# sshaoshuai/PointRCNN

Measured on NVIDIA B200. Metric: scenes/sec RPN backbone fwd (16384 pts), higher is better.
Workload: dtype f32 (tf32 tensor-core MLP, fp32 accumulate)

## Files before the change

include/pointrcnn_b200.h:

```cpp
#ifndef POINTRCNN_B200_H_
#define POINTRCNN_B200_H_

#include <stddef.h>
#include <stdint.h>

#ifdef __cplusplus
extern "C" {
#endif

#define PRB_ABI_VERSION 5
#if defined(__GNUC__)
#define PRB_API __attribute__((visibility("default")))
#else
#define PRB_API
#endif

PRB_API int prb_abi_version(void);
PRB_API const char *prb_last_error(void);
PRB_API unsigned long long prb_launch_count(void);

typedef struct prb_options {
    int fps_cluster;
    int fps_prune;
    int fps_threads;
// ... 78 lines not shown

PRB_API size_t prb_mlp_packed_bytes(int num_layers, int c_in, const int *c_out);
PRB_API int prb_mlp_pack_weights(int num_layers, int c_in, const int *c_out, const float *const *w, void *dst);

PRB_API int prb_sa_group_mlp_max(int b, int n, int npoint, int nsample, int c_feat, const float *xyz,
                         const float *new_xyz, const float *feats_pm, const int *idx,
                         const prb_mlp_desc *mlp, float *out, int out_stride_c, int out_c_off,
                         void *stream);

PRB_API int prb_fp_interp_mlp(int b, int n, int m, int c_known, int c_skip, const float *known_pm,
                      const int *idx, const float *weight, const float *skip,
                      const prb_mlp_desc *mlp, float *out, void *stream);

PRB_API size_t prb_mlp_packed_bytes_ex(int kind, int split, int num_layers, int c_in, const int *c_out);
PRB_API int prb_mlp_pack_weights_ex(int kind, int split, int num_layers, int c_in, const int *c_out,
                                    const float *const *w, void *dst);
PRB_API size_t prb_sa_workspace_bytes(int b, int npoint, int nsample, int c_feat, int num_layers, const int *c_out);
PRB_API size_t prb_fp_workspace_bytes(int b, int n, int c_known, int c_skip, int num_layers, const int *c_out);
PRB_API size_t prb_rows_workspace_bytes(long rows, int c_in, int num_layers, const int *c_out);
PRB_API int prb_sa_group_mlp_max_ws(int b, int n, int npoint, int nsample, int c_feat, const float *xyz,
                                    const float *new_xyz, const float *feats_pm, const int *idx,
                                    const prb_mlp_desc *mlp, float *out, float *out_pm, int out_stride_c,
                                    int out_c_off, void *workspace, size_t workspace_bytes, void *stream);
PRB_API int prb_fp_interp_mlp_ws(int b, int n, int m, int c_known, int c_skip, const float *known_pm,
                                 const int *idx, const float *weight, const float *skip,
                                 const prb_mlp_desc *mlp, float *out, float *out_pm, void *workspace,
                                 size_t workspace_bytes, void *stream);
PRB_API int prb_mlp_rows(long rows, int c_in, const float *x_rows, const prb_mlp_desc *mlp, float *out_rows,
                         int out_pitch, void *workspace, size_t workspace_bytes, void *stream);
PRB_API size_t prb_rows2_workspace_bytes(long rows, int c_a, int c_b, int num_layers, const int *c_out);
PRB_API int prb_mlp_rows2(long rows, int c_a, const float *a_rows, int a_pitch, int c_b, const float *b_rows, int b_pitch,
                          const prb_mlp_desc *mlp, float *out_rows, int out_pitch, void *workspace, size_t workspace_bytes,
                          void *stream);

PRB_API int prb_decode_rpn_proposals(long n, int c, const float *xyz, const float *reg, const float *anchor_hwl,
                                     float loc_scope, float loc_bin_size, int num_head_bin, int get_xz_fine, float *out,
                                     void *stream);
PRB_API size_t prb_rpn_proposals_workspace_bytes(int b, int post_nms_top_n);
PRB_API int prb_rpn_proposals(int b, int n, const float *boxes, const float *scores, const long long *order,
                              int distance_based, int pre_nms_top_n, int post_nms_top_n, float nms_thresh, int normal_nms,
                              float *out_boxes, float *out_scores, void *workspace, size_t workspace_bytes, void *stream);

PRB_API int prb_debug_mlp_trace(long long *dst);
PRB_API int prb_debug_pipe_trace(long long *dst);
PRB_API int prb_debug_tuned_plans(int *dst, int max_entries);

// ... 53 lines not shown
```

pointrcnn_b200/csrc/mlp_dev.cuh:

```cuda
#pragma once
#include <math_constants.h>

#include "common.cuh"

namespace prb {

constexpr int TM = 128;
constexpr int KC = 32;
constexpr int A_STAGE_BYTES = TM * KC * 4;
constexpr int B_TILE_ROWS = 256;
constexpr int MAX_STAGES = 4;
constexpr int MAX_LAYERS = 3;
constexpr int MAX_NP = 512;

enum { IN_SA = 0, IN_FP = 1, IN_DIRECT = 2 };
enum { OUT_ROWS = 0, OUT_SA_MAX = 1, OUT_FP = 2 };

struct ChainParams {
    int mode_in, mode_out, num_layers;
    int nchunks[MAX_LAYERS];
    int np[MAX_LAYERS];
    int dcol[MAX_LAYERS];
    const float *w[MAX_LAYERS];
    const float *scale[MAX_LAYERS];
    int w_resident;
    int sleepy_ns;
    int sleepy;
    int a_tmem;
    int trace;
    int unit_scale;
    const float *shift[MAX_LAYERS];
    int na, nb;
    int b_stage_bytes;
    int tmem_cols;
    int gather_mode;
    int linear_last;
    int round_out;
    int nseg, seg_chunks[2], seg_width[2];
    long total_rows;
    int num_tiles;
    int n, npoint, ns, log_ns, c_feat;
    const float *xyz, *new_xyz, *feats_pm;
    const int *idx;
    int m, c_known, c_skip;
    const float *known_pm, *weight, *skip;
    const float *x_rows;
    int x_pitch;
    const float *x2_rows;
    int x2_pitch;
    float *out;
    float *out_pm;
    int c_last;
    int out_stride_c, out_c_off, out_pitch;
    int rcol[MAX_LAYERS];
    int zcol[2], zs, nslice, nbuf;
    int nb0, nb1;
    int b0_stage_bytes, b1_stage_bytes;
    int b_rows;
    int nsplit, split_w;
    int num_items;
    int rows32;
    int pool_mode;
};

__device__ __forceinline__ uint32_t s2u(const void *p) { return (uint32_t)__cvta_generic_to_shared(p); }

// ... 191 lines not shown
```

pointrcnn_b200/csrc/mlp_pipe.cu:

```cuda
#include <type_traits>

#include <map>
#include <mutex>

#include "mlp_dev.cuh"

namespace prb {

constexpr int PIPE_MAX_A = 8;
constexpr int PIPE_MAX_B = 12;

struct PipeSmem {
    uint64_t a_full[PIPE_MAX_A], a_empty[PIPE_MAX_A];
    uint64_t b0_full[PIPE_MAX_B], b0_empty[PIPE_MAX_B], b1_full[PIPE_MAX_B], b1_empty[PIPE_MAX_B];
    uint64_t r_full[2];
    uint64_t x_free;
    uint64_t ready[2][16];
    uint64_t z_full[2], z_free[2];
    uint32_t tmem_base;
    int row_src[2][TM][3];
    float row_aux[2][TM][3];
    int row_valid[2][TM];
};

__host__ __device__ inline size_t pipe_smem_bytes(int ne, int na, int nb0, int b0_bytes, int nb1, int b1_bytes, int np_total, bool pool) {
    return 1024  + (size_t)na * A_STAGE_BYTES + (size_t)nb0 * b0_bytes + (size_t)nb1 * b1_bytes +
           (size_t)2 * np_total * sizeof(float) + (pool ? (size_t)ne * (TM * POOL_STRIDE + 8 * 16) * sizeof(float) : 0) + 64;
}

__device__ __forceinline__ void bar_named(int id, int nthreads) {
    asm volatile("bar.sync %0, %1;" ::"r"(id), "r"(nthreads) : "memory");
}

struct Cursor {
    int scene, pos, adv_scene, adv_pos, period;
    __device__ __forceinline__ void init(int start, int step, int per) {
        period = per;
        scene = start / per; pos = start - scene * per;
        adv_scene = step / per; adv_pos = step - adv_scene * per;
    }
    __device__ __forceinline__ void advance() {
        scene += adv_scene; pos += adv_pos;
        if (pos >= period) { pos -= period; ++scene; }
    }
    __device__ __forceinline__ void at(int off, int &sc, int &ps) const {
        sc = scene; ps = pos + off;
        while (ps >= period) { ps -= period; ++sc; }
    }
};

// ... 149 lines not shown
template <int BASE, int N>
__device__ __forceinline__ void reg_set() {
    if (N > BASE) asm volatile("setmaxnreg.inc.sync.aligned.u32 %0;" ::"n"(N));
    else if (N < BASE) asm volatile("setmaxnreg.dec.sync.aligned.u32 %0;" ::"n"(N));
}

template <int NE, int NGW, int MINB, int MIN, int MOUT>
__global__ void __launch_bounds__((NE + NGW + 1) * 128, MINB) mlp_pipe_kernel(const __grid_constant__ ChainParams p) {
    constexpr int NTHREADS = (NE + NGW + 1) * 128;
    constexpr int REG_BASE = (65536 / (NTHREADS * MINB)) / 8 * 8 > 255 ? 255 : (65536 / (NTHREADS * MINB)) / 8 * 8;
    static_assert(128 * (RegPlan<NE, NGW, MINB>::MISC + NE * RegPlan<NE, NGW, MINB>::EPI + NGW * RegPlan<NE, NGW, MINB>::GATHER) <= NTHREADS * REG_BASE,
                  "register plan exceeds the CTA's launch allocation");
    constexpr int W_GATHER = 4 * NE, W_MISC = 4 * (NE + NGW);
    extern __shared__ uint8_t smem_raw[];
    __shared__ PipeSmem S;
    uint8_t *base = smem_raw + ((1024u - (s2u(smem_raw) & 1023u)) & 1023u);
    const int L = p.num_layers;
    auto sc_off = [&](int l) { return l == 0 ? 0 : (l == 1 ? p.np[0] : p.np[0] + p.np[1]); };
    static_assert(MAX_LAYERS == 3, "sc_off assumes at most three layers");
    const int np_total = sc_off(L - 1) + p.np[L - 1];
    uint8_t *sA = base;
    uint8_t *sB0 = sA + (size_t)p.na * A_STAGE_BYTES;
    uint8_t *sB1 = sB0 + (size_t)p.nb0 * p.b0_stage_bytes;
    float *s_scale = reinterpret_cast<float *>(sB1 + (size_t)p.nb1 * p.b1_stage_bytes);
    float *s_shift = s_scale + np_total;
    float *s_pool = s_shift + np_total;
    const int tid = threadIdx.x, warp = tid >> 5, lane = tid & 31;

    if (tid == 0) {
        for (int i = 0; i < PIPE_MAX_A; ++i) { mbar_init(s2u(&S.a_full[i]), 128); mbar_init(s2u(&S.a_empty[i]), 1); }
        for (int i = 0; i < PIPE_MAX_B; ++i) {
            mbar_init(s2u(&S.b0_full[i]), 1); mbar_init(s2u(&S.b0_empty[i]), 1);
            mbar_init(s2u(&S.b1_full[i]), 1); mbar_init(s2u(&S.b1_empty[i]), 1);
        }
        for (int i = 0; i < 2; ++i) {
            mbar_init(s2u(&S.r_full[i]), 1);
            mbar_init(s2u(&S.z_full[i]), 1); mbar_init(s2u(&S.z_free[i]), 128 * NE);
            for (int k = 0; k < 16; ++k) mbar_init(s2u(&S.ready[i][k]), 128);
        }
        mbar_init(s2u(&S.x_free), 1);
        asm volatile("fence.mbarrier_init.release.cluster;" ::: "memory");
    }
    if (warp == W_MISC + 2) tmem_alloc(s2u(&S.tmem_base), (uint32_t)p.tmem_cols);
    for (int l = 0; l < L; ++l)
        for (int i = tid; i < p.np[l]; i += NTHREADS) { s_scale[sc_off(l) + i] = p.unit_scale ? 1.f : p.scale[l][i]; s_shift[sc_off(l) + i] = p.shift[l][i]; }
    tc_fence_before();
    __syncthreads();
    tc_fence_after();
    const uint32_t tmem = S.tmem_base;
    const int brows = p.b_rows;
    const int nsplit = p.nsplit;
    const int sj = (int)blockIdx.x % nsplit;
    const int tile0 = (int)blockIdx.x / nsplit, tstep = (int)gridDim.x / nsplit;
    const int ntiles = p.num_tiles;
    const bool resident = p.w_resident != 0;
    const int lazy = NE == 1 ? p.sleepy_ns : 0;
    TraceTimer tt;
    tt.start(p.trace != 0 && blockIdx.x == 0 && (warp >= W_MISC || warp == W_GATHER || warp == 0),
             warp == W_MISC + 2 ? 0 : warp == W_MISC + 3 ? 1 : warp == W_MISC ? 2 : warp == W_MISC + 1 ? 3 : warp == W_GATHER ? 4 : 5);

    if (warp >= W_MISC) {
    reg_set<REG_BASE, RegPlan<NE, NGW, MINB>::MISC>();
    if (warp == W_MISC) {
        {
            RingPos rb = {0, 0};
            const int col0 = sj * p.split_w;
            const int width = L == 1 ? min(p.split_w, p.np[0] - col0) : p.np[0];
            const int halves = (width + brows - 1) / brows;
// ... 144 lines not shown
                                        }
                                    }
                                });
                                rb.advance(nb);
                            }
                        }
                    }
                }
            }
        }
    }
    } else if (warp >= W_GATHER) {
        reg_set<REG_BASE, RegPlan<NE, NGW, MINB>::GATHER>();
        const int gw = warp - W_GATHER;
        const int wq = gw & 3, grp = gw >> 2;
        const int r = wq * 32 + lane;
        const int j8 = lane & 7;
        const int rsub = lane >> 3;
        const int na = p.na, nch0 = p.nchunks[0];
        const int rows = p.rows32;
        RingPos ra = {0, 0};
        uint32_t cc = 0, it = 0;
        Cursor cur;
        if (MIN == IN_SA) cur.init(tile0 * (TM >> p.log_ns), tstep * (TM >> p.log_ns), p.npoint);
        else if (MIN == IN_FP) cur.init(tile0 * TM, tstep * TM, p.n);
        else cur.init(0, 0, 1);
        for (int tile = tile0; tile < ntiles; tile += tstep, ++it, cur.advance()) {
            const int R = tile * TM + r;
            const bool valid = R < rows;
            int src = -1;
            float cx = 0.f, cy = 0.f, cz = 0.f;
            int my_scene = 0, my_u = 0;
            const int par = it & 1;
            if (MIN == IN_SA) {
                int sc, pp;
                cur.at(r >> p.log_ns, sc, pp);
                if (valid) {
                    src = sc * p.n + __ldg(p.idx + R);
                    const float *ctr = p.new_xyz + ((size_t)sc * p.npoint + pp) * 3;
                    cx = __ldg(ctr); cy = __ldg(ctr + 1); cz = __ldg(ctr + 2);
                }
            } else if (MIN == IN_FP) {
                cur.at(r, my_scene, my_u);
                int m_src[3] = {0, 0, 0};
                float m_w[3] = {0.f, 0.f, 0.f};
                if (valid) {
#pragma unroll
                    for (int q = 0; q < 3; ++q) {
                        m_src[q] = my_scene * p.m + __ldg(p.idx + (size_t)R * 3 + q);
                        m_w[q] = __ldg(p.weight + (size_t)R * 3 + q);
                    }
                }
                if (grp == 0) {
                    S.row_valid[par][r] = valid;
#pragma unroll
                    for (int q = 0; q < 3; ++q) { S.row_src[par][r][q] = m_src[q]; S.row_aux[par][r][q] = m_w[q]; }
                }
                bar_named(5, 128 * NGW);
            }
            int s8[8];
            if (MIN == IN_SA) {
#pragma unroll
                for (int i = 0; i < 8; ++i) s8[i] = __shfl_sync(0xffffffffu, src, rsub + 4 * i);
            } else if (MIN == IN_DIRECT) {
#pragma unroll
                for (int i = 0; i < 8; ++i) { const int rr = tile * TM + wq * 32 + rsub + 4 * i; s8[i] = rr < rows ? rr : -1; }
            }

            for (int kc = 0; kc < nch0; ++kc, ++cc, ra.advance(na)) {
                if (NGW > 1 && (int)(cc % NGW) != grp) continue;
                int c = kc, seg = 0;
                if (p.nseg > 1 && c >= p.seg_chunks[0]) { c -= p.seg_chunks[0]; seg = 1; }
                const int k0 = c * KC;
                const int width = p.seg_width[seg];
                uint8_t *A = sA + (size_t)ra.stage * A_STAGE_BYTES;
                uint64_t *empty_bar = &S.a_empty[ra.stage];
                const uint32_t empty_par = ra.phase ^ 1;
                const bool rows_seg = (MIN == IN_DIRECT) || (MIN == IN_SA && seg == 0 && p.c_feat > 5) || (MIN == IN_FP && seg == 0);
                if (rows_seg) {
                    const int kk = k0 + 4 * j8;
                    if (MIN == IN_FP) {
// ... 48 lines not shown
                        for (int i = 0; i < 8; ++i) {
                            t[i] = make_float4(0.f, 0.f, 0.f, 0.f);
                            if (s8[i] >= 0 && kk < width) {
                                const float *sp = srcbase + (size_t)s8[i] * pitch + kk;
                                if (vec) {
                                    t[i] = __ldg((const float4 *)sp);
                                } else {
                                    float o[4];
#pragma unroll
                                    for (int q = 0; q < 4; ++q) o[q] = (kk + q < width) ? __ldg(sp + q) : 0.f;
                                    t[i] = make_float4(o[0], o[1], o[2], o[3]);
                                }
                            }
                        }
                        tt.timed(0, [&] { bwait_lazy(empty_bar, empty_par, lazy); });
#pragma unroll
                        for (int i = 0; i < 8; ++i) {
                            const int rr = wq * 32 + rsub + 4 * i;
                            float4 v = t[i];
                            v.x = to_tf32(v.x); v.y = to_tf32(v.y); v.z = to_tf32(v.z); v.w = to_tf32(v.w);
                            *reinterpret_cast<float4 *>(A + swz(rr, j8)) = v;
                        }
                    }
                } else if (MIN == IN_SA) {
                    float4 v = make_float4(0.f, 0.f, 0.f, 0.f), v2 = make_float4(0.f, 0.f, 0.f, 0.f);
                    if (valid) {
                        const float *q = p.xyz + (size_t)src * 3;
                        v.x = to_tf32(__ldg(q + 0) - cx);
                        v.y = to_tf32(__ldg(q + 1) - cy);
                        v.z = to_tf32(__ldg(q + 2) - cz);
                        const int cf = p.c_feat;
                        if (cf > 0 && cf <= 5) {
                            const float *f = p.feats_pm + (size_t)src * cf;
                            v.w = to_tf32(__ldg(f));
                            if (cf > 1) v2.x = to_tf32(__ldg(f + 1));
                            if (cf > 2) v2.y = to_tf32(__ldg(f + 2));
                            if (cf > 3) v2.z = to_tf32(__ldg(f + 3));
                            if (cf > 4) v2.w = to_tf32(__ldg(f + 4));
                        }
                    }
                    tt.timed(0, [&] { bwait_lazy(empty_bar, empty_par, lazy); });
                    *reinterpret_cast<float4 *>(A + swz(r, 0)) = v;
                    *reinterpret_cast<float4 *>(A + swz(r, 1)) = v2;
                } else if (MIN == IN_FP) {
                    const float *bsrc = p.skip + (size_t)my_scene * p.c_skip * p.n + my_u;
                    float o[32];
// ... 397 lines not shown
            if (o.mlp_ne == 2) { pl.ne = pl.ngw = 2; pl.occ = 1; }
            if (pl.ne == 2 && (o.mlp_ngw == 3 || force_ngw == 3)) pl.ngw = 3;
            const int brows = o.mlp_brows >= 32 ? o.mlp_brows : 256;
            pl.brows = brows;
            int b0_rows = L == 1 ? z : p.np[0], b1_rows = 32;
            for (int l = 1; l < L; ++l) { const int w = (l == L - 1) ? z : p.np[l]; if (w > b1_rows) b1_rows = w; }
            if (b0_rows > brows) b0_rows = brows;
            if (b1_rows > brows) b1_rows = brows;
            pl.b0_bytes = b0_rows * KC * 4; pl.b1_bytes = L > 1 ? b1_rows * KC * 4 : 0;
            const size_t budget = (size_t)(227 * 1024) / pl.occ - 1024 - sizeof(PipeSmem) - 512;
            bool ok = false;
            pl.resident = 0;
            if (o.mlp_resident) {
                const int halves0 = ((L == 1 ? z : p.np[0]) + brows - 1) / brows;
                int st0 = p.nchunks[0] * halves0, st1 = 0;
                for (int l = 1; l < L; ++l) {
                    const int w = (l == L - 1) ? z : p.np[l];
                    st1 += (l == L - 1 ? nslice : 1) * p.nchunks[l] * ((w + brows - 1) / brows);
                }
                if (st0 <= PIPE_MAX_B && st1 <= PIPE_MAX_B) {
                    const int na_min = k0 + 1 < PIPE_MAX_A ? (k0 + 1 > 3 ? k0 + 1 : 3) : PIPE_MAX_A;
                    for (int na = (k0 + 2 < PIPE_MAX_A ? (k0 + 2 > 3 ? k0 + 2 : 3) : PIPE_MAX_A); na >= na_min && !ok; --na) {
                        const size_t smem = pipe_smem_bytes(pl.ne, na, st0, pl.b0_bytes, st1, pl.b1_bytes, np_total,
                                                            p.mode_out == OUT_SA_MAX && !(p.ns == 16 || p.ns == 32));
                        if (smem <= budget && smem <= (size_t)max_optin) {
                            pl.na = na; pl.nb0 = st0; pl.nb1 = st1; pl.smem = smem; pl.resident = 1; ok = true;
                        }
                    }
                }
            }
            for (int nb = 3; nb >= 2 && !ok; --nb)
                for (int na = (k0 + 2 < PIPE_MAX_A ? (k0 + 2 > 3 ? k0 + 2 : 3) : PIPE_MAX_A); na >= 2 && !ok; --na) {
                    const size_t smem = pipe_smem_bytes(pl.ne, na, nb, pl.b0_bytes, L > 1 ? nb : 0, pl.b1_bytes, np_total,
                                                        p.mode_out == OUT_SA_MAX && !(p.ns == 16 || p.ns == 32));
                    if (smem <= budget && smem <= (size_t)max_optin && (nb == 2 || na >= (k0 < 4 ? k0 : 4))) {
                        pl.na = na; pl.nb0 = nb; pl.nb1 = L > 1 ? nb : 0; pl.smem = smem; ok = true;
                    }
                }
            if (!ok) continue;
            const long score = (long)pl.occ * 1000000L + nbuf * 1000L + z;
            if (score > best_score) { best_score = score; best = pl; }
        }
    }
    if (best_score < 0) return false;
    *out = best;
    return true;
}

static int launch_with_plan(ChainParams &p, const PipePlan &pl, cudaStream_t st) {
    const int L = p.num_layers;
    int col = 0;
    for (int l = 0; l + 1 < L; ++l) { p.rcol[l] = col; col += p.np[l]; }
    p.zcol[0] = col; p.zcol[1] = col + pl.zs;
    p.zs = pl.zs; p.nslice = pl.nslice; p.nbuf = pl.nbuf;
    p.tmem_cols = pl.cols;
    p.na = pl.na; p.nb0 = pl.nb0; p.nb1 = pl.nb1 > 0 ? pl.nb1 : 1;
    p.b0_stage_bytes = pl.b0_bytes; p.b1_stage_bytes = pl.b1_bytes;
    p.nsplit = pl.nsplit; p.split_w = pl.split_w;
    p.b_rows = pl.brows;
    p.w_resident = pl.resident;
    p.num_items = p.num_tiles * pl.nsplit;
    int sms = num_sms();
    if (const int v = opts().mlp_sms; v >= 1 && v < sms) sms = v;
    int grid = sms * pl.occ;
    if (grid > p.num_items) grid = p.num_items;
    grid = grid / pl.nsplit * pl.nsplit;
    if (grid < pl.nsplit) grid = pl.nsplit;
    p.trace = opts().mlp_trace ? 1 : 0;
    p.rows32 = (int)p.total_rows;
    p.pool_mode = opts().mlp_pool;
    p.sleepy_ns = opts().mlp_lazy_ns > 0 ? opts().mlp_lazy_ns : 400;
    const size_t smem = pl.smem;
#define PRB_LAUNCH_PIPE(NE, NGW, MB, MI, MO)                                                                                   \
    do {                                                                                                                       \
        PRB_CUDA(cudaFuncSetAttribute(mlp_pipe_kernel<NE, NGW, MB, MI, MO>, cudaFuncAttributeMaxDynamicSharedMemorySize, (int)smem)); \
        mlp_pipe_kernel<NE, NGW, MB, MI, MO><<<grid, (NE + NGW + 1) * 128, smem, st>>>(p);                                      \
    } while (0)
#define PRB_LAUNCH_PIPE_IO(NE, NGW, MB)                                                                    \
    do {                                                                                                   \
        const int key = p.mode_in * 3 + p.mode_out;                                                        \
        switch (key) {                                                                                     \
            case IN_SA * 3 + OUT_ROWS: PRB_LAUNCH_PIPE(NE, NGW, MB, IN_SA, OUT_ROWS); break;              \
            case IN_SA * 3 + OUT_SA_MAX: PRB_LAUNCH_PIPE(NE, NGW, MB, IN_SA, OUT_SA_MAX); break;          \
            case IN_FP * 3 + OUT_ROWS: PRB_LAUNCH_PIPE(NE, NGW, MB, IN_FP, OUT_ROWS); break;              \
            case IN_FP * 3 + OUT_FP: PRB_LAUNCH_PIPE(NE, NGW, MB, IN_FP, OUT_FP); break;                  \
            case IN_DIRECT * 3 + OUT_ROWS: PRB_LAUNCH_PIPE(NE, NGW, MB, IN_DIRECT, OUT_ROWS); break;      \
            case IN_DIRECT * 3 + OUT_SA_MAX: PRB_LAUNCH_PIPE(NE, NGW, MB, IN_DIRECT, OUT_SA_MAX); break;  \
            case IN_DIRECT * 3 + OUT_FP: PRB_LAUNCH_PIPE(NE, NGW, MB, IN_DIRECT, OUT_FP); break;          \
            default: set_error("mlp: unsupported input / output mode pair %d / %d", p.mode_in, p.mode_out); return -1; \
        }                                                                                                  \
    } while (0)
    if (pl.occ == 3) PRB_LAUNCH_PIPE(1, 1, 3, IN_SA, OUT_SA_MAX);
    else if (pl.ne == 1 && pl.ngw == 1) PRB_LAUNCH_PIPE_IO(1, 1, 2);
    else if (pl.ngw == 3) PRB_LAUNCH_PIPE_IO(2, 3, 1);
    else PRB_LAUNCH_PIPE_IO(2, 2, 1);
#undef PRB_LAUNCH_PIPE_IO
#undef PRB_LAUNCH_PIPE
    return check_launch("mlp_pipe_kernel");
}

struct TuneKey {
    int dev, mode_in, mode_out, L, ns, k0, tiles, np[3];
    bool operator<(const TuneKey &o) const { return memcmp(this, &o, sizeof(TuneKey)) < 0; }
};
static std::mutex g_tune_mu;
struct TuneVal { int choice; int nc; int code[4]; float ms[4]; };
static std::map<TuneKey, TuneVal> g_tune;

static bool tuning_allowed(cudaStream_t st) {
    const prb_options &o = opts();
    if (!o.mlp_tune || o.mlp_trace || o.mlp_occ || o.mlp_ne || o.mlp_ngw || o.mlp_zs || o.mlp_nbuf) return false;
    cudaStreamCaptureStatus cs = cudaStreamCaptureStatusNone;
    if (cudaStreamIsCapturing(st, &cs) != cudaSuccess) { cudaGetLastError(); return false; }
    return cs == cudaStreamCaptureStatusNone;
}

int launch_chain_pipe(ChainParams &p, cudaStream_t st) {
    int max_optin = 0, dev = 0;
    PRB_CUDA(cudaGetDevice(&dev));
    PRB_CUDA(cudaDeviceGetAttribute(&max_optin, cudaDevAttrMaxSharedMemoryPerBlockOptin, dev));
    p.num_tiles = (int)((p.total_rows + TM - 1) / TM);
    if (p.num_tiles == 0) return 0;
    PipePlan pl;
    if (!(opts().mlp_occ == 3 && pipe_plan(p, max_optin, &pl, 3, 0)))
        PRB_REQUIRE(pipe_plan(p, max_optin, &pl), "mlp: no tensor-memory / shared-memory plan for this chain segment");
    PipePlan cand[4];
    int code[4], nc = 0;
    cand[nc] = pl; code[nc++] = pl.occ == 2 ? 2 : (pl.ngw == 3 ? 3 : 1);
    if (pl.occ == 2 && opts().mlp_occ != 2 && pipe_plan(p, max_optin, &cand[nc], 3, 0)) code[nc++] = 4;
    if (pl.occ == 2 && pipe_plan(p, max_optin, &cand[nc], 1, 0)) code[nc++] = 1;
    if (pl.ngw != 3 && pipe_plan(p, max_optin, &cand[nc], 1, 3) && cand[nc].ngw == 3) code[nc++] = 3;
    if (nc > 1) {
        TuneKey key;
        memset(&key, 0, sizeof(key));
        key.dev = dev; key.mode_in = p.mode_in; key.mode_out = p.mode_out; key.L = p.num_layers; key.ns = p.ns;
        key.k0 = p.nchunks[0]; key.tiles = p.num_tiles;
        for (int l = 0; l < p.num_layers; ++l) key.np[l] = p.np[l];
        int choice = 0;
        {
            std::lock_guard<std::mutex> g(g_tune_mu);
            auto it = g_tune.find(key);
            if (it != g_tune.end()) choice = it->second.choice;
        }
        if (choice == 0 && tuning_allowed(st)) {
            cudaEvent_t e0, e1;
            PRB_CUDA(cudaEventCreate(&e0));
            PRB_CUDA(cudaEventCreate(&e1));
            float best[4] = {1e30f, 1e30f, 1e30f, 1e30f};
            int rc = 0;
            for (int c = 0; c < nc && !rc; ++c)
                for (int rep = 0; rep < 3 && !rc; ++rep) {
                    ChainParams q = p;
                    cudaEventRecord(e0, st);
                    rc = launch_with_plan(q, cand[c], st);
                    cudaEventRecord(e1, st);
                    if (cudaEventSynchronize(e1) != cudaSuccess) rc = rc ? rc : -1;
                    float ms = 0.f;
                    cudaEventElapsedTime(&ms, e0, e1);
// ... 6 lines not shown
            for (int c = 1; c < nc; ++c)
                if (best[c] < 0.97f * best[win]) win = c;
            choice = code[win];
            TuneVal tv;
            memset(&tv, 0, sizeof(tv));
            tv.choice = choice; tv.nc = nc;
            for (int c = 0; c < nc; ++c) { tv.code[c] = code[c]; tv.ms[c] = best[c]; }
            std::lock_guard<std::mutex> g(g_tune_mu);
            g_tune[key] = tv;
        }
        for (int c = 0; c < nc; ++c)
            if (code[c] == choice) pl = cand[c];
    }
    return launch_with_plan(p, pl, st);
}

int pipe_tuned_plans(int *dst, int max_entries) {
    std::lock_guard<std::mutex> g(g_tune_mu);
    int n = 0;
    for (const auto &kv : g_tune) {
        if (n >= max_entries) break;
        const TuneKey &k = kv.first;
        int *d = dst + 18 * n++;
        d[0] = k.mode_in; d[1] = k.mode_out; d[2] = k.L; d[3] = k.ns; d[4] = k.k0; d[5] = k.tiles; d[6] = k.np[0]; d[7] = k.np[1]; d[8] = k.np[2];
        d[9] = kv.second.choice;
        for (int c = 0; c < 4; ++c) {
            d[10 + 2 * c] = c < kv.second.nc ? kv.second.code[c] : 0;
            d[11 + 2 * c] = c < kv.second.nc ? (int)(kv.second.ms[c] * 1000.f + 0.5f) : 0;
        }
    }
    return n;
}

}

extern "C" int prb_debug_tuned_plans(int *dst, int max_entries) { return prb::pipe_tuned_plans(dst, max_entries); }

extern "C" int prb_debug_pipe_trace(long long *dst) {
    PRB_CUDA(cudaDeviceSynchronize());
    PRB_CUDA(cudaMemcpyFromSymbol(dst, prb::g_pipe_trace, sizeof(long long) * 64));
    static long long zeros[64];
    PRB_CUDA(cudaMemcpyToSymbol(prb::g_pipe_trace, zeros, sizeof(zeros)));
    return 0;
}
```

pointrcnn_b200/csrc/mlp_tc.cu:

```cuda
#include <string.h>

#include <vector>

#include "mlp_dev.cuh"

namespace prb {

__device__ long long g_trace[32 * 16];
#define PRB_TRACE(slot) do { if (p.trace && blockIdx.x == 0 && tcount < 32 && r == 0) g_trace[tcount * 16 + (slot)] = clock64(); } while (0)

template <int NG, int MINB>
__global__ void __launch_bounds__(128 * NG + 64, MINB) mlp_chain_kernel(const ChainParams p) {
    constexpr int NTHREADS = 128 * NG + 64;
    extern __shared__ uint8_t smem_raw[];
    __shared__ SmemFixed S;
    uint8_t *base = smem_raw + ((1024u - (s2u(smem_raw) & 1023u)) & 1023u);
    const int L = p.num_layers;
    int np_total = 0, sc_off[MAX_LAYERS];
    for (int l = 0; l < L; ++l) { sc_off[l] = np_total; np_total += p.np[l]; }
    uint8_t *sA = base;
    uint8_t *sB = sA + (size_t)p.na * A_STAGE_BYTES;
    float *s_scale = reinterpret_cast<float *>(sB + (size_t)p.nb * p.b_stage_bytes);
    float *s_shift = s_scale + np_total;
    float *s_pool = s_shift + np_total;
// ... 856 lines not shown
}

PRB_API int prb_sa_group_mlp_max_ws(int b, int n, int npoint, int nsample, int c_feat, const float *xyz, const float *new_xyz,
                                    const float *feats_pm, const int *idx, const prb_mlp_desc *mlp, float *out, float *out_pm,
                                    int out_stride_c, int out_c_off, void *workspace, size_t workspace_bytes, void *stream) {
    PRB_REQUIRE(b >= 0 && n > 0 && npoint > 0 && nsample > 0 && xyz && new_xyz && idx && mlp && out, "sa_group_mlp_max: bad arguments");
    PRB_REQUIRE(mlp->c_in == 3 + c_feat, "sa_group_mlp_max: c_in %d != 3 + c_feat %d", mlp->c_in, c_feat);
    PRB_REQUIRE(c_feat == 0 || feats_pm, "sa_group_mlp_max: features missing");
    PRB_REQUIRE(nsample >= 4 && nsample <= 128 && (nsample & (nsample - 1)) == 0, "sa_group_mlp_max: nsample %d must be a power of two in [4,128]", nsample);
    if (b == 0) return 0;
    ChainIO io;
    memset(&io, 0, sizeof(io));
    io.kind = 0; io.split = c_feat;
    io.rows = (long)b * npoint * nsample;
    io.base.mode_in = IN_SA; io.base.mode_out = OUT_SA_MAX;
    io.base.n = n; io.base.npoint = npoint; io.base.ns = nsample; io.base.c_feat = c_feat;
    io.base.log_ns = 0;
    while ((1 << io.base.log_ns) < nsample) ++io.base.log_ns;
    io.base.xyz = xyz; io.base.new_xyz = new_xyz; io.base.feats_pm = feats_pm; io.base.idx = idx;
    io.base.out = out; io.base.out_pm = out_pm; io.base.out_stride_c = out_stride_c; io.base.out_c_off = out_c_off;
    return run_chain(io, mlp, workspace, workspace_bytes, (cudaStream_t)stream);
}

PRB_API int prb_fp_interp_mlp_ws(int b, int n, int m, int c_known, int c_skip, const float *known_pm, const int *idx,
                                 const float *weight, const float *skip, const prb_mlp_desc *mlp, float *out, float *out_pm,
                                 void *workspace, size_t workspace_bytes, void *stream) {
    PRB_REQUIRE(b >= 0 && n > 0 && m > 0 && c_known > 0 && known_pm && idx && weight && mlp && out, "fp_interp_mlp: bad arguments");
    PRB_REQUIRE(mlp->c_in == c_known + c_skip, "fp_interp_mlp: c_in %d != %d + %d", mlp->c_in, c_known, c_skip);
    PRB_REQUIRE(c_skip == 0 || skip, "fp_interp_mlp: skip features missing");
    if (b == 0) return 0;
    ChainIO io;
    memset(&io, 0, sizeof(io));
    io.kind = 1; io.split = c_known;
    io.rows = (long)b * n;
    io.base.mode_in = IN_FP; io.base.mode_out = OUT_FP;
    io.base.n = n; io.base.m = m; io.base.c_known = c_known; io.base.c_skip = c_skip;
    io.base.known_pm = known_pm; io.base.idx = idx; io.base.weight = weight; io.base.skip = skip;
    io.base.out = out; io.base.out_pm = out_pm; io.base.out_stride_c = mlp->c_out[mlp->num_layers - 1]; io.base.out_c_off = 0;
    return run_chain(io, mlp, workspace, workspace_bytes, (cudaStream_t)stream);
}

PRB_API int prb_mlp_rows(long rows, int c_in, const float *x_rows, const prb_mlp_desc *mlp, float *out_rows, int out_pitch,
                         void *workspace, size_t workspace_bytes, void *stream) {
    PRB_REQUIRE(rows >= 0 && c_in > 0 && x_rows && mlp && out_rows, "mlp_rows: bad arguments");
    PRB_REQUIRE(mlp->c_in == c_in, "mlp_rows: c_in mismatch");
    const int np_last = (mlp->c_out[mlp->num_layers - 1] + 31) / 32 * 32;
// ... 50 lines not shown
```

pointrcnn_b200/pointnet2/pointnet2_modules.py:

```python
import ctypes
from typing import List

import numpy as np
import torch
import torch.nn as nn
import torch.nn.functional as F

from .. import _cabi as C
from .. import config
from .. import prof
from . import pointnet2_utils
from . import pytorch_utils as pt_utils


def _round_up(a, b):
    return (a + b - 1) // b * b


class _FusedMLP:

    def __init__(self):
        self.key = None
        self.desc = None
        self.tensors = None
        self.c_out = None

    @staticmethod
    def supported(mlp: nn.Sequential):
        layers = list(mlp.children())
        if not 1 <= len(layers) <= 3:
            return False
        for layer in layers:
            names = [k for k, _ in layer.named_children()]
            if names not in (["conv", "bn", "activation"], ["conv", "activation"]):
                return False
            if not isinstance(layer.activation, nn.ReLU):
                return False
            conv = layer.conv
            if tuple(conv.kernel_size) not in ((1, 1), (1,)) or conv.out_channels > 512:
                return False
            if "bn" in names and layer.bn.bn.training:
                return False
        return True

    def get(self, mlp: nn.Sequential, kind: int, split: int, device, project_known: bool = False):
        layers = list(mlp.children())
        tensors = []
        for layer in layers:
            tensors += [layer.conv.weight, layer.conv.bias]
            if hasattr(layer, "bn"):
                bn = layer.bn.bn
                tensors += [bn.weight, bn.bias, bn.running_mean, bn.running_var]
        key = (kind, split, str(device), _fold_scale(), project_known) + tuple((id(t), t._version) if t is not None else None for t in tensors)
        if key == self.key:
            return self.desc
        L = len(layers)
        c_in = layers[0].conv.in_channels
        c_out = [layer.conv.out_channels for layer in layers]
        ws, scales, shifts = [], [], []
        with torch.no_grad():
            for layer in layers:
                conv = layer.conv
                W = conv.weight.detach().reshape(conv.out_channels, -1).float().cpu().contiguous()
                co = conv.out_channels
                if hasattr(layer, "bn"):
                    bn = layer.bn.bn
                    inv = (bn.weight.detach().float() / torch.sqrt(bn.running_var.detach().float() + bn.eps)).cpu()
                    sh = (bn.bias.detach().float().cpu() - bn.running_mean.detach().float().cpu() * inv)
                    if conv.bias is not None:
                        sh = sh + inv * conv.bias.detach().float().cpu()
                else:
                    inv = torch.ones(co)
                    sh = conv.bias.detach().float().cpu() if conv.bias is not None else torch.zeros(co)
                pad = _round_up(co, 32) - co
                if _fold_scale():
                    W = (W * inv[:, None]).contiguous()
                ws.append(W)
                scales.append(F.pad(inv, (0, pad)))
                shifts.append(F.pad(sh, (0, pad)))
        lib = C.lib()
        self.proj = None
        if project_known:
            W0 = ws[0]
            c1, c_known = W0.shape[0], split
            self.proj = self._pack(lib, 2, 0, c_known, [c1], [W0[:, :c_known].contiguous()], torch.zeros(_round_up(c1, 32)), device, flags=1)
            ws[0] = torch.cat([torch.eye(c1), W0[:, c_known:]], dim=1).contiguous()
            c_in, split = c1 + (c_in - c_known), c1
        co_arr = (ctypes.c_int * 3)(*(c_out + [0] * (3 - L)))
        nbytes = lib.prb_mlp_packed_bytes_ex(kind, split, L, c_in, co_arr)
        host = np.zeros(nbytes // 4, dtype=np.float32)
        wp = (ctypes.c_void_p * L)(*[w.data_ptr() for w in ws])
        C.check(lib.prb_mlp_pack_weights_ex(kind, split, L, c_in, co_arr, wp, host.ctypes.data_as(ctypes.c_void_p)), "mlp_pack")
        packed = torch.from_numpy(host).to(device)
        scale = torch.cat(scales).contiguous().to(device)
        shift = torch.cat(shifts).contiguous().to(device)
        desc = C.MlpDesc()
        desc.num_layers, desc.c_in = L, c_in
        for i in range(3):
            desc.c_out[i] = c_out[i] if i < L else 0
        desc.packed_w, desc.scale, desc.shift = packed.data_ptr(), (None if _fold_scale() else scale.data_ptr()), shift.data_ptr()
        self.key, self.desc, self.tensors, self.c_out = key, desc, (packed, scale, shift), c_out
        return desc

    @staticmethod
    def _pack(lib, kind, split, c_in, c_out, ws, shift, device, flags=0):
        L = len(ws)
        co_arr = (ctypes.c_int * 3)(*(c_out + [0] * (3 - L)))
        nbytes = lib.prb_mlp_packed_bytes_ex(kind, split, L, c_in, co_arr)
        host = np.zeros(nbytes // 4, dtype=np.float32)
        wp = (ctypes.c_void_p * L)(*[w.data_ptr() for w in ws])
        C.check(lib.prb_mlp_pack_weights_ex(kind, split, L, c_in, co_arr, wp, host.ctypes.data_as(ctypes.c_void_p)), "mlp_pack")
        packed = torch.from_numpy(host).to(device)
        shift = shift.contiguous().to(device)
        desc = C.MlpDesc()
        desc.num_layers, desc.c_in = L, c_in
        for i in range(3):
            desc.c_out[i] = c_out[i] if i < L else 0
        desc.packed_w, desc.scale, desc.shift, desc.flags = packed.data_ptr(), None, shift.data_ptr(), flags
        return dict(desc=desc, keep=(packed, shift, ws), c_out=c_out, co_arr=co_arr)


def _attach_pm(t, pm):
    t._prb_pm = (pm, t._version)
    return t


def _point_major(t):
    twin = getattr(t, "_prb_pm", None)
    if twin is not None and twin[1] == t._version and twin[0].shape == (t.size(0), t.size(2), t.size(1)) and twin[0].device == t.device:
        return twin[0]
    return pointnet2_utils.transpose_bcn_to_bnc(t.contiguous())


def rows_mlp(fused: "_FusedMLP", mlp: nn.Sequential, a: torch.Tensor, b: torch.Tensor = None, tag="rows_mlp"):
    lib = C.lib()
    dev = a.device
    rows, c_a = a.shape
    c_b = 0 if b is None else b.size(1)
    assert a.stride(1) == 1 and (b is None or (b.stride(1) == 1 and b.size(0) == rows))
    desc = fused.get(mlp, 1 if c_b else 2, c_a if c_b else 0, dev)
    c_out = fused.c_out
    pitch = _round_up(c_out[-1], 32)
# ... 69 lines not shown
        if self.npoint is None:
            centres = torch.zeros((B, 1, 3), dtype=torch.float32, device=dev)
            ar = torch.arange(N, dtype=torch.int32, device=dev).view(1, 1, N).expand(B, 1, N).contiguous()
            return None, centres, [ar for _ in self.groupers], [N for _ in self.groupers]
        if new_xyz is None:
            _, new_xyz = pointnet2_utils.furthest_point_sample_xyz(xyz, self.npoint)
        centres = new_xyz.contiguous()
        if len(self.groupers) == 2:
            g0, g1 = self.groupers
            idxs = list(pointnet2_utils.ball_query_msg2((g0.radius, g1.radius), (g0.nsample, g1.nsample), xyz, centres))
        else:
            idxs = [pointnet2_utils.ball_query(g.radius, g.nsample, xyz, centres) for g in self.groupers]
        return new_xyz, centres, idxs, [g.nsample for g in self.groupers]

    def fused_mlp(self, xyz, features, centres, idxs, nss):
        lib = C.lib()
        B, N, _ = xyz.shape
        dev = xyz.device
        npoint = centres.size(1)
        c_feat = 0 if features is None else features.size(1)
        feats_pm = _point_major(features) if features is not None else None
        if self._fused is None or len(self._fused) != len(self.mlps):
            self._fused = [_FusedMLP() for _ in self.mlps]
        descs = [f.get(mlp, 0, c_feat, dev) for f, mlp in zip(self._fused, self.mlps)]
        c_total = sum(f.c_out[-1] for f in self._fused)
        out = torch.empty((B, c_total, npoint), dtype=torch.float32, device=dev)
        out_pm = torch.empty((B, npoint, c_total), dtype=torch.float32, device=dev)
        off = 0
        with torch.cuda.device(dev):
            for desc, fused, idx, ns in zip(descs, self._fused, idxs, nss):
                co_arr = (ctypes.c_int * 3)(*(fused.c_out + [0] * (3 - len(fused.c_out))))
                wsb = lib.prb_sa_workspace_bytes(B, npoint, ns, c_feat, desc.num_layers, co_arr)
                ws = torch.empty(wsb, dtype=torch.uint8, device=dev)
                with prof.region("sa_mlp", "%dx%d [%d]+%s" % (B * npoint, ns, 3 + c_feat, fused.c_out)):
                    C.check(lib.prb_sa_group_mlp_max_ws(B, N, npoint, ns, c_feat, C.ptr(xyz), C.ptr(centres), C.ptr(feats_pm),
                                                        C.ptr(idx), ctypes.byref(desc), C.ptr(out), C.ptr(out_pm), out.size(1), off,
                                                        C.ptr(ws), C.c_size_t(wsb), C.stream()), "sa_group_mlp_max")
                off += fused.c_out[-1]
        return _attach_pm(out, out_pm)

    def _forward_fused(self, xyz, features, new_xyz):
        xyz = xyz.contiguous()
        ret_xyz, centres, idxs, nss = self.fused_geometry(xyz, new_xyz)
        return ret_xyz, self.fused_mlp(xyz, features, centres, idxs, nss)

    def forward(self, xyz: torch.Tensor, features: torch.Tensor = None, new_xyz=None) -> (torch.Tensor, torch.Tensor):
        if self._can_fuse(xyz, features, new_xyz):
            return self._forward_fused(xyz, features, new_xyz)

        new_features_list = []
        if new_xyz is None and self.npoint is not None:
            xyz_flipped = xyz.transpose(1, 2).contiguous()
            new_xyz = pointnet2_utils.gather_operation(
# ... 133 lines not shown
```

Baseline: 9123.

## Compute first SA layer on CUDA cores inside the pipelined producer

```diff
diff --git a/include/pointrcnn_b200.h b/include/pointrcnn_b200.h
--- a/include/pointrcnn_b200.h
+++ b/include/pointrcnn_b200.h
@@ -124,6 +124,10 @@
                                     const float *new_xyz, const float *feats_pm, const int *idx,
                                     const prb_mlp_desc *mlp, float *out, float *out_pm, int out_stride_c,
                                     int out_c_off, void *workspace, size_t workspace_bytes, void *stream);
+PRB_API int prb_sa_group_mlp_max_l0(int b, int n, int npoint, int nsample, int c_feat, const float *xyz,
+                                    const float *new_xyz, const float *feats_pm, const int *idx, int c0,
+                                    const float *l0_w, const float *l0_shift, const prb_mlp_desc *mlp, float *out,
+                                    float *out_pm, int out_stride_c, int out_c_off, void *stream);
 PRB_API int prb_fp_interp_mlp_ws(int b, int n, int m, int c_known, int c_skip, const float *known_pm,
                                  const int *idx, const float *weight, const float *skip,
                                  const prb_mlp_desc *mlp, float *out, float *out_pm, void *workspace,
diff --git a/pointrcnn_b200/csrc/mlp_dev.cuh b/pointrcnn_b200/csrc/mlp_dev.cuh
--- a/pointrcnn_b200/csrc/mlp_dev.cuh
+++ b/pointrcnn_b200/csrc/mlp_dev.cuh
@@ -14,6 +14,8 @@
 constexpr int MAX_NP = 512;
 
 enum { IN_SA = 0, IN_FP = 1, IN_DIRECT = 2 };
+enum { IN_SA_L0 = 3 };
+constexpr int L0_IN = 8;
 enum { OUT_ROWS = 0, OUT_SA_MAX = 1, OUT_FP = 2 };
 
 struct ChainParams {
@@ -42,6 +44,8 @@
     int n, npoint, ns, log_ns, c_feat;
     const float *xyz, *new_xyz, *feats_pm;
     const int *idx;
+    int sa_l0, l0_c, l0_np;
+    const float *l0_w, *l0_shift;
     int m, c_known, c_skip;
     const float *known_pm, *weight, *skip;
     const float *x_rows;
diff --git a/pointrcnn_b200/csrc/mlp_pipe.cu b/pointrcnn_b200/csrc/mlp_pipe.cu
--- a/pointrcnn_b200/csrc/mlp_pipe.cu
+++ b/pointrcnn_b200/csrc/mlp_pipe.cu
@@ -23,9 +23,17 @@
     int row_valid[2][TM];
 };
 
-__host__ __device__ inline size_t pipe_smem_bytes(int ne, int na, int nb0, int b0_bytes, int nb1, int b1_bytes, int np_total, bool pool) {
+__host__ __device__ inline size_t pipe_smem_bytes(int ne, int na, int nb0, int b0_bytes, int nb1, int b1_bytes, int np_total, bool pool,
+                                                  int l0_np) {
     return 1024  + (size_t)na * A_STAGE_BYTES + (size_t)nb0 * b0_bytes + (size_t)nb1 * b1_bytes +
-           (size_t)2 * np_total * sizeof(float) + (pool ? (size_t)ne * (TM * POOL_STRIDE + 8 * 16) * sizeof(float) : 0) + 64;
+           (size_t)l0_np * (L0_IN + 1) * sizeof(float) + (size_t)2 * np_total * sizeof(float) +
+           (pool ? (size_t)ne * (TM * POOL_STRIDE + 8 * 16) * sizeof(float) : 0) + 64;
+}
+
+__device__ __forceinline__ float tf32_rna_bits(float x) {
+    uint32_t u = __float_as_uint(x);
+    if ((u & 0x7f800000u) != 0x7f800000u) u += 0x1000u;
+    return __uint_as_float(u & 0xffffe000u);
 }
 
 __device__ __forceinline__ void bar_named(int id, int nthreads) {
@@ -221,7 +229,9 @@
     uint8_t *sA = base;
     uint8_t *sB0 = sA + (size_t)p.na * A_STAGE_BYTES;
     uint8_t *sB1 = sB0 + (size_t)p.nb0 * p.b0_stage_bytes;
-    float *s_scale = reinterpret_cast<float *>(sB1 + (size_t)p.nb1 * p.b1_stage_bytes);
+    float *s_l0w = reinterpret_cast<float *>(sB1 + (size_t)p.nb1 * p.b1_stage_bytes);
+    float *s_l0sh = s_l0w + (size_t)p.l0_np * L0_IN;
+    float *s_scale = s_l0sh + p.l0_np;
     float *s_shift = s_scale + np_total;
     float *s_pool = s_shift + np_total;
     const int tid = threadIdx.x, warp = tid >> 5, lane = tid & 31;
@@ -243,6 +253,10 @@
     if (warp == W_MISC + 2) tmem_alloc(s2u(&S.tmem_base), (uint32_t)p.tmem_cols);
     for (int l = 0; l < L; ++l)
         for (int i = tid; i < p.np[l]; i += NTHREADS) { s_scale[sc_off(l) + i] = p.unit_scale ? 1.f : p.scale[l][i]; s_shift[sc_off(l) + i] = p.shift[l][i]; }
+    if (MIN == IN_SA_L0) {
+        for (int i = tid; i < p.l0_np * L0_IN; i += NTHREADS) s_l0w[i] = (i / L0_IN) < p.l0_c ? tf32_rna_bits(p.l0_w[i]) : 0.f;
+        for (int i = tid; i < p.l0_np; i += NTHREADS) s_l0sh[i] = i < p.l0_c ? p.l0_shift[i] : 0.f;
+    }
     tc_fence_before();
     __syncthreads();
     tc_fence_after();
@@ -433,7 +447,7 @@
         RingPos ra = {0, 0};
         uint32_t cc = 0, it = 0;
         Cursor cur;
-        if (MIN == IN_SA) cur.init(tile0 * (TM >> p.log_ns), tstep * (TM >> p.log_ns), p.npoint);
+        if (MIN == IN_SA || MIN == IN_SA_L0) cur.init(tile0 * (TM >> p.log_ns), tstep * (TM >> p.log_ns), p.npoint);
         else if (MIN == IN_FP) cur.init(tile0 * TM, tstep * TM, p.n);
         else cur.init(0, 0, 1);
         for (int tile = tile0; tile < ntiles; tile += tstep, ++it, cur.advance()) {
@@ -443,7 +457,7 @@
             float cx = 0.f, cy = 0.f, cz = 0.f;
             int my_scene = 0, my_u = 0;
             const int par = it & 1;
-            if (MIN == IN_SA) {
+            if (MIN == IN_SA || MIN == IN_SA_L0) {
                 int sc, pp;
                 cur.at(r >> p.log_ns, sc, pp);
                 if (valid) {
@@ -468,6 +482,22 @@
                     for (int q = 0; q < 3; ++q) { S.row_src[par][r][q] = m_src[q]; S.row_aux[par][r][q] = m_w[q]; }
                 }
                 bar_named(5, 128 * NGW);
+            }
+            float in0[L0_IN];
+            if (MIN == IN_SA_L0) {
+#pragma unroll
+                for (int k = 0; k < L0_IN; ++k) in0[k] = 0.f;
+                if (valid) {
+                    const float *q = p.xyz + (size_t)src * 3;
+                    in0[0] = to_tf32(__ldg(q + 0) - cx);
+                    in0[1] = to_tf32(__ldg(q + 1) - cy);
+                    in0[2] = to_tf32(__ldg(q + 2) - cz);
+                    const int cf = p.c_feat;
+                    const float *f = p.feats_pm + (size_t)src * cf;
+#pragma unroll
+                    for (int k = 0; k < L0_IN - 3; ++k)
+                        if (k < cf) in0[3 + k] = to_tf32(__ldg(f + k));
+                }
             }
             int s8[8];
             if (MIN == IN_SA) {
@@ -562,6 +592,38 @@
                             *reinterpret_cast<float4 *>(A + swz(rr, j8)) = v;
                         }
                     }
+                } else if (MIN == IN_SA_L0) {
+                    tt.timed(0, [&] { bwait_lazy(empty_bar, empty_par, lazy); });
+                    const float4 *w4 = reinterpret_cast<const float4 *>(s_l0w + (size_t)k0 * L0_IN);
+                    const float4 *sh4 = reinterpret_cast<const float4 *>(s_l0sh + k0);
+                    auto chunk = [&](auto wide_c) {
+                        constexpr bool WIDE = decltype(wide_c)::value;
+#pragma unroll
+                        for (int j = 0; j < 8; ++j) {
+                            const float4 b = sh4[j];
+                            float o[4];
+#pragma unroll
+                            for (int q = 0; q < 4; ++q) {
+                                const float4 wa = w4[2 * (4 * j + q)];
+                                float acc = __fmul_rn(wa.x, in0[0]);
+                                acc = __fmaf_rn(wa.y, in0[1], acc);
+                                acc = __fmaf_rn(wa.z, in0[2], acc);
+                                acc = __fmaf_rn(wa.w, in0[3], acc);
+                                if (WIDE) {
+                                    const float4 wb = w4[2 * (4 * j + q) + 1];
+                                    acc = __fmaf_rn(wb.x, in0[4], acc);
+                                    acc = __fmaf_rn(wb.y, in0[5], acc);
+                                    acc = __fmaf_rn(wb.z, in0[6], acc);
+                                    acc = __fmaf_rn(wb.w, in0[7], acc);
+                                }
+                                const float t = q == 0 ? b.x : q == 1 ? b.y : q == 2 ? b.z : b.w;
+                                o[q] = valid ? relu_to_tf32(acc + t) : 0.f;
+                            }
+                            *reinterpret_cast<float4 *>(A + swz(r, j)) = make_float4(o[0], o[1], o[2], o[3]);
+                        }
+                    };
+                    if (p.c_feat > 1) chunk(std::true_type{});
+                    else chunk(std::false_type{});
                 } else if (MIN == IN_SA) {
                     float4 v = make_float4(0.f, 0.f, 0.f, 0.f), v2 = make_float4(0.f, 0.f, 0.f, 0.f);
                     if (valid) {
@@ -1005,7 +1067,7 @@
                     const int na_min = k0 + 1 < PIPE_MAX_A ? (k0 + 1 > 3 ? k0 + 1 : 3) : PIPE_MAX_A;
                     for (int na = (k0 + 2 < PIPE_MAX_A ? (k0 + 2 > 3 ? k0 + 2 : 3) : PIPE_MAX_A); na >= na_min && !ok; --na) {
                         const size_t smem = pipe_smem_bytes(pl.ne, na, st0, pl.b0_bytes, st1, pl.b1_bytes, np_total,
-                                                            p.mode_out == OUT_SA_MAX && !(p.ns == 16 || p.ns == 32));
+                                                            p.mode_out == OUT_SA_MAX && !(p.ns == 16 || p.ns == 32), p.sa_l0 ? p.l0_np : 0);
                         if (smem <= budget && smem <= (size_t)max_optin) {
                             pl.na = na; pl.nb0 = st0; pl.nb1 = st1; pl.smem = smem; pl.resident = 1; ok = true;
                         }
@@ -1015,7 +1077,8 @@
             for (int nb = 3; nb >= 2 && !ok; --nb)
                 for (int na = (k0 + 2 < PIPE_MAX_A ? (k0 + 2 > 3 ? k0 + 2 : 3) : PIPE_MAX_A); na >= 2 && !ok; --na) {
                     const size_t smem = pipe_smem_bytes(pl.ne, na, nb, pl.b0_bytes, L > 1 ? nb : 0, pl.b1_bytes, np_total,
-                                                        p.mode_out == OUT_SA_MAX && !(p.ns == 16 || p.ns == 32));
+                                                        p.mode_out == OUT_SA_MAX && !(p.ns == 16 || p.ns == 32),
+                                                        p.sa_l0 ? p.l0_np : 0);
                     if (smem <= budget && smem <= (size_t)max_optin && (nb == 2 || na >= (k0 < 4 ? k0 : 4))) {
                         pl.na = na; pl.nb0 = nb; pl.nb1 = L > 1 ? nb : 0; pl.smem = smem; ok = true;
                     }
@@ -1061,10 +1124,11 @@
     } while (0)
 #define PRB_LAUNCH_PIPE_IO(NE, NGW, MB)                                                                    \
     do {                                                                                                   \
-        const int key = p.mode_in * 3 + p.mode_out;                                                        \
+        const int key = (p.sa_l0 ? IN_SA_L0 : p.mode_in) * 3 + p.mode_out;                                \
         switch (key) {                                                                                     \
             case IN_SA * 3 + OUT_ROWS: PRB_LAUNCH_PIPE(NE, NGW, MB, IN_SA, OUT_ROWS); break;              \
             case IN_SA * 3 + OUT_SA_MAX: PRB_LAUNCH_PIPE(NE, NGW, MB, IN_SA, OUT_SA_MAX); break;          \
+            case IN_SA_L0 * 3 + OUT_SA_MAX: PRB_LAUNCH_PIPE(NE, NGW, MB, IN_SA_L0, OUT_SA_MAX); break;    \
             case IN_FP * 3 + OUT_ROWS: PRB_LAUNCH_PIPE(NE, NGW, MB, IN_FP, OUT_ROWS); break;              \
             case IN_FP * 3 + OUT_FP: PRB_LAUNCH_PIPE(NE, NGW, MB, IN_FP, OUT_FP); break;                  \
             case IN_DIRECT * 3 + OUT_ROWS: PRB_LAUNCH_PIPE(NE, NGW, MB, IN_DIRECT, OUT_ROWS); break;      \
@@ -1073,7 +1137,8 @@
             default: set_error("mlp: unsupported input / output mode pair %d / %d", p.mode_in, p.mode_out); return -1; \
         }                                                                                                  \
     } while (0)
-    if (pl.occ == 3) PRB_LAUNCH_PIPE(1, 1, 3, IN_SA, OUT_SA_MAX);
+    if (pl.occ == 3 && p.sa_l0) PRB_LAUNCH_PIPE(1, 1, 3, IN_SA_L0, OUT_SA_MAX);
+    else if (pl.occ == 3) PRB_LAUNCH_PIPE(1, 1, 3, IN_SA, OUT_SA_MAX);
     else if (pl.ne == 1 && pl.ngw == 1) PRB_LAUNCH_PIPE_IO(1, 1, 2);
     else if (pl.ngw == 3) PRB_LAUNCH_PIPE_IO(2, 3, 1);
     else PRB_LAUNCH_PIPE_IO(2, 2, 1);
@@ -1116,7 +1181,7 @@
     if (nc > 1) {
         TuneKey key;
         memset(&key, 0, sizeof(key));
-        key.dev = dev; key.mode_in = p.mode_in; key.mode_out = p.mode_out; key.L = p.num_layers; key.ns = p.ns;
+        key.dev = dev; key.mode_in = p.sa_l0 ? IN_SA_L0 : p.mode_in; key.mode_out = p.mode_out; key.L = p.num_layers; key.ns = p.ns;
         key.k0 = p.nchunks[0]; key.tiles = p.num_tiles;
         for (int l = 0; l < p.num_layers; ++l) key.np[l] = p.np[l];
         int choice = 0;
@@ -1169,7 +1234,8 @@
         if (n >= max_entries) break;
         const TuneKey &k = kv.first;
         int *d = dst + 18 * n++;
-        d[0] = k.mode_in; d[1] = k.mode_out; d[2] = k.L; d[3] = k.ns; d[4] = k.k0; d[5] = k.tiles; d[6] = k.np[0]; d[7] = k.np[1]; d[8] = k.np[2];
+        d[0] = k.mode_in == IN_SA_L0 ? IN_SA : k.mode_in;
+        d[1] = k.mode_out; d[2] = k.L; d[3] = k.ns; d[4] = k.k0; d[5] = k.tiles; d[6] = k.np[0]; d[7] = k.np[1]; d[8] = k.np[2];
         d[9] = kv.second.choice;
         for (int c = 0; c < 4; ++c) {
             d[10 + 2 * c] = c < kv.second.nc ? kv.second.code[c] : 0;
diff --git a/pointrcnn_b200/csrc/mlp_tc.cu b/pointrcnn_b200/csrc/mlp_tc.cu
--- a/pointrcnn_b200/csrc/mlp_tc.cu
+++ b/pointrcnn_b200/csrc/mlp_tc.cu
@@ -902,6 +902,37 @@
     return run_chain(io, mlp, workspace, workspace_bytes, (cudaStream_t)stream);
 }
 
+PRB_API int prb_sa_group_mlp_max_l0(int b, int n, int npoint, int nsample, int c_feat, const float *xyz, const float *new_xyz,
+                                    const float *feats_pm, const int *idx, int c0, const float *l0_w, const float *l0_shift,
+                                    const prb_mlp_desc *mlp, float *out, float *out_pm, int out_stride_c, int out_c_off, void *stream) {
+    PRB_REQUIRE(b >= 0 && n > 0 && npoint > 0 && nsample > 0 && xyz && new_xyz && idx && mlp && out && l0_w && l0_shift,
+                "sa_group_mlp_max_l0: bad arguments");
+    PRB_REQUIRE(c_feat >= 0 && c_feat <= L0_IN - 3, "sa_group_mlp_max_l0: c_feat %d > %d", c_feat, L0_IN - 3);
+    PRB_REQUIRE(c_feat == 0 || feats_pm, "sa_group_mlp_max_l0: features missing");
+    PRB_REQUIRE(c0 >= 1 && c0 <= MAX_NP && mlp->c_in == c0, "sa_group_mlp_max_l0: layer-0 width %d / chain input %d", c0, mlp->c_in);
+    PRB_REQUIRE(mlp->scale == nullptr, "sa_group_mlp_max_l0: the BN scale must be folded into the weights");
+    PRB_REQUIRE(nsample >= 4 && nsample <= 128 && (nsample & (nsample - 1)) == 0, "sa_group_mlp_max_l0: nsample %d must be a power of two in [4,128]", nsample);
+    PRB_REQUIRE(use_pipe(), "sa_group_mlp_max_l0: needs the pipelined kernel (mlp_pipeline = 1, mlp_gather = 0)");
+    const int L = mlp->num_layers;
+    PRB_REQUIRE(L >= 1 && L <= MAX_LAYERS, "sa_group_mlp_max_l0: num_layers %d unsupported", L);
+    LayerGeom g[MAX_LAYERS];
+    chain_geometry(L, 1, &c0, mlp->c_out, g, nullptr);
+    PRB_REQUIRE(fits_pipe(g, 0, L), "sa_group_mlp_max_l0: the chain does not fit one launch");
+    if (b == 0) return 0;
+    ChainIO io;
+    memset(&io, 0, sizeof(io));
+    io.kind = 2; io.split = 0;
+    io.rows = (long)b * npoint * nsample;
+    io.base.mode_in = IN_SA; io.base.mode_out = OUT_SA_MAX;
+    io.base.sa_l0 = 1; io.base.l0_c = c0; io.base.l0_np = round_up(c0, KC); io.base.l0_w = l0_w; io.base.l0_shift = l0_shift;
+    io.base.n = n; io.base.npoint = npoint; io.base.ns = nsample; io.base.c_feat = c_feat;
+    io.base.log_ns = 0;
+    while ((1 << io.base.log_ns) < nsample) ++io.base.log_ns;
+    io.base.xyz = xyz; io.base.new_xyz = new_xyz; io.base.feats_pm = feats_pm; io.base.idx = idx;
+    io.base.out = out; io.base.out_pm = out_pm; io.base.out_stride_c = out_stride_c; io.base.out_c_off = out_c_off;
+    return run_chain(io, mlp, nullptr, 0, (cudaStream_t)stream);
+}
+
 PRB_API int prb_fp_interp_mlp_ws(int b, int n, int m, int c_known, int c_skip, const float *known_pm, const int *idx,
                                  const float *weight, const float *skip, const prb_mlp_desc *mlp, float *out, float *out_pm,
                                  void *workspace, size_t workspace_bytes, void *stream) {
diff --git a/pointrcnn_b200/pointnet2/pointnet2_modules.py b/pointrcnn_b200/pointnet2/pointnet2_modules.py
--- a/pointrcnn_b200/pointnet2/pointnet2_modules.py
+++ b/pointrcnn_b200/pointnet2/pointnet2_modules.py
@@ -24,6 +24,8 @@
         self.desc = None
         self.tensors = None
         self.c_out = None
+        self.proj = None
+        self.l0 = None
 
     @staticmethod
     def supported(mlp: nn.Sequential):
@@ -43,7 +45,7 @@
                 return False
         return True
 
-    def get(self, mlp: nn.Sequential, kind: int, split: int, device, project_known: bool = False):
+    def get(self, mlp: nn.Sequential, kind: int, split: int, device, project_known: bool = False, layer0: bool = False):
         layers = list(mlp.children())
         tensors = []
         for layer in layers:
@@ -51,7 +53,7 @@
             if hasattr(layer, "bn"):
                 bn = layer.bn.bn
                 tensors += [bn.weight, bn.bias, bn.running_mean, bn.running_var]
-        key = (kind, split, str(device), _fold_scale(), project_known) + tuple((id(t), t._version) if t is not None else None for t in tensors)
+        key = (kind, split, str(device), _fold_scale(), project_known, layer0) + tuple((id(t), t._version) if t is not None else None for t in tensors)
         if key == self.key:
             return self.desc
         L = len(layers)
@@ -80,13 +82,23 @@
                 shifts.append(F.pad(sh, (0, pad)))
         lib = C.lib()
         self.proj = None
+        self.l0 = None
+        if layer0:
+            assert _fold_scale() and L >= 2 and kind == 0 and c_in == 3 + split <= L0_IN
+            w0, sh0 = split_layer0(ws[0], shifts[0][:c_out[0]])
+            self.l0 = dict(w=w0.to(device), shift=sh0.to(device), c0=c_out[0])
+            ws, scales, shifts = ws[1:], scales[1:], shifts[1:]
+            kind, split, c_in, L = 2, 0, c_out[0], L - 1
+            c_out_chain = c_out[1:]
+        else:
+            c_out_chain = c_out
         if project_known:
             W0 = ws[0]
             c1, c_known = W0.shape[0], split
             self.proj = self._pack(lib, 2, 0, c_known, [c1], [W0[:, :c_known].contiguous()], torch.zeros(_round_up(c1, 32)), device, flags=1)
             ws[0] = torch.cat([torch.eye(c1), W0[:, c_known:]], dim=1).contiguous()
             c_in, split = c1 + (c_in - c_known), c1
-        co_arr = (ctypes.c_int * 3)(*(c_out + [0] * (3 - L)))
+        co_arr = (ctypes.c_int * 3)(*(c_out_chain + [0] * (3 - L)))
         nbytes = lib.prb_mlp_packed_bytes_ex(kind, split, L, c_in, co_arr)
         host = np.zeros(nbytes // 4, dtype=np.float32)
         wp = (ctypes.c_void_p * L)(*[w.data_ptr() for w in ws])
@@ -97,7 +109,7 @@
         desc = C.MlpDesc()
         desc.num_layers, desc.c_in = L, c_in
         for i in range(3):
-            desc.c_out[i] = c_out[i] if i < L else 0
+            desc.c_out[i] = c_out_chain[i] if i < L else 0
         desc.packed_w, desc.scale, desc.shift = packed.data_ptr(), (None if _fold_scale() else scale.data_ptr()), shift.data_ptr()
         self.key, self.desc, self.tensors, self.c_out = key, desc, (packed, scale, shift), c_out
         return desc
@@ -118,6 +130,32 @@
             desc.c_out[i] = c_out[i] if i < L else 0
         desc.packed_w, desc.scale, desc.shift, desc.flags = packed.data_ptr(), None, shift.data_ptr(), flags
         return dict(desc=desc, keep=(packed, shift, ws), c_out=c_out, co_arr=co_arr)
+
+
+L0_IN = 8
+
+
+def split_layer0(w0: torch.Tensor, shift0: torch.Tensor):
+    c0, c_in = w0.shape
+    assert c_in <= L0_IN and shift0.shape == (c0,)
+    w = torch.zeros((c0, L0_IN), dtype=torch.float32)
+    w[:, :c_in] = w0.float()
+    return w.contiguous(), shift0.float().contiguous()
+
+
+def _layer0_direct(mlp: nn.Sequential, c_feat: int) -> bool:
+    if c_feat > L0_IN - 3 or not _fold_scale():
+        return False
+    c_out = [layer.conv.out_channels for layer in mlp.children()]
+    if len(c_out) < 2:
+        return False
+    np_ = [_round_up(c, 32) for c in c_out[1:]]
+    last = np_[-1]
+    if last > 512 or sum(np_[:-1]) + (2 * min(last, 64) if len(np_) > 1 else 0) > 512:
+        return False
+    o = C.Options()
+    C.lib().prb_get_thread_options(ctypes.byref(o))
+    return o.mlp_pipeline != 0 and o.mlp_gather == 0
 
 
 def _attach_pm(t, pm):
@@ -233,13 +271,22 @@
         feats_pm = _point_major(features) if features is not None else None
         if self._fused is None or len(self._fused) != len(self.mlps):
             self._fused = [_FusedMLP() for _ in self.mlps]
-        descs = [f.get(mlp, 0, c_feat, dev) for f, mlp in zip(self._fused, self.mlps)]
+        direct = [_layer0_direct(mlp, c_feat) for mlp in self.mlps]
+        descs = [f.get(mlp, 0, c_feat, dev, layer0=d) for f, mlp, d in zip(self._fused, self.mlps, direct)]
         c_total = sum(f.c_out[-1] for f in self._fused)
         out = torch.empty((B, c_total, npoint), dtype=torch.float32, device=dev)
         out_pm = torch.empty((B, npoint, c_total), dtype=torch.float32, device=dev)
         off = 0
         with torch.cuda.device(dev):
             for desc, fused, idx, ns in zip(descs, self._fused, idxs, nss):
+                if fused.l0 is not None:
+                    l0 = fused.l0
+                    with prof.region("sa_mlp", "%dx%d [%d]+%s l0" % (B * npoint, ns, 3 + c_feat, fused.c_out)):
+                        C.check(lib.prb_sa_group_mlp_max_l0(B, N, npoint, ns, c_feat, C.ptr(xyz), C.ptr(centres), C.ptr(feats_pm),
+                                                            C.ptr(idx), l0["c0"], C.ptr(l0["w"]), C.ptr(l0["shift"]), ctypes.byref(desc),
+                                                            C.ptr(out), C.ptr(out_pm), out.size(1), off, C.stream()), "sa_group_mlp_max_l0")
+                    off += fused.c_out[-1]
+                    continue
                 co_arr = (ctypes.c_int * 3)(*(fused.c_out + [0] * (3 - len(fused.c_out))))
                 wsb = lib.prb_sa_workspace_bytes(B, npoint, ns, c_feat, desc.num_layers, co_arr)
                 ws = torch.empty(wsb, dtype=torch.uint8, device=dev)
```

Result: faster. 9540 (median of 6 runs) (+4.6%).
